# see--/speech_recognition

Hardware: AMD Instinct MI355X
Metric: 1s 16kHz clips/sec training throughput (higher is better)
Workload: dtype f32

## Files before the change

speech_recognition_amd/csrc/dw_bwd_body.h:

```cpp
#pragma once
#include "internal.h"

namespace kws_dw {

#ifndef KWS_DW_NT
#define KWS_DW_NT 1
#endif
typedef float dw_v4f __attribute__((ext_vector_type(4)));
__device__ __forceinline__ float4 ld4_stream(const float* p) {
  if (KWS_DW_NT & 2) {
    const dw_v4f v = __builtin_nontemporal_load(reinterpret_cast<const dw_v4f*>(p));
    return make_float4(v.x, v.y, v.z, v.w);
  }
  return *reinterpret_cast<const float4*>(p);
}
__device__ __forceinline__ void st4_stream(float* p, float4 o) {
  if (KWS_DW_NT & 1) {
    dw_v4f v = {o.x, o.y, o.z, o.w};
    __builtin_nontemporal_store(v, reinterpret_cast<dw_v4f*>(p));
    return;
  }
  *reinterpret_cast<float4*>(p) = o;
}

#ifndef KWS_DW_TT
#define KWS_DW_TT 8
#endif
constexpr int TT = KWS_DW_TT;

__device__ __forceinline__ float4 f4_fma(float4 a, float4 b, float4 c) {
  return make_float4(fmaf(a.x, b.x, c.x), fmaf(a.y, b.y, c.y), fmaf(a.z, b.z, c.z), fmaf(a.w, b.w, c.w));
}
__device__ __forceinline__ float4 f4_mul(float4 a, float4 b) {
  return make_float4(a.x * b.x, a.y * b.y, a.z * b.z, a.w * b.w);
}
__device__ __forceinline__ float4 f4_zero() { return make_float4(0.f, 0.f, 0.f, 0.f); }

#ifndef DW_BWD_THREADS
#define DW_BWD_THREADS 512
#endif
#ifndef DW_BWD_HT
#define DW_BWD_HT 8
#endif
#ifndef DW_BWD2_THREADS
#define DW_BWD2_THREADS 512
#endif
#ifndef DW_BWD_PARTS
#define DW_BWD_PARTS 256
#endif

struct BwdArgs {
  const float* dz; const float* y; const float* bn; const float* w; const float* coef;
  float* g; float* part;
  int B, Lin, Lout, C, pad_l, nchunks, R, Cb;
  unsigned* amax;
  int add_stride = 0, add_len = 0;
};
constexpr int bwd_smem_floats(int mode, int threads) { return mode == 2 ? 4 : 5 * threads * 4; }

template <int S, bool HAS_BN, int MODE, bool GUARD, bool ADDS = false>
__device__ __forceinline__ void bwd_body(const BwdArgs& p, float* const red, const int bid, const int nblk, const int by) {
  const float* __restrict__ dz = p.dz;
  const float* __restrict__ y = p.y;
  const float* __restrict__ bn = p.bn;
  const float* __restrict__ w = p.w;
  const float* __restrict__ coef = p.coef;
  float* __restrict__ g = p.g;
  float* __restrict__ part = p.part;
  const int B = p.B, Lin = p.Lin, Lout = p.Lout, C = p.C, pad_l = p.pad_l, nchunks = p.nchunks, R = p.R, Cb = p.Cb;
  constexpr int RSTRIDE = (MODE == 2 ? 4 : DW_BWD_THREADS * 4);
  float gmax = 0.f;
  const int C4 = Cb >> 2;
  const int tid = threadIdx.x;
  const bool live = !GUARD || tid < R * C4;
  const int r = live ? tid / C4 : 0, c4 = live ? tid - r * C4 : 0;
  const int c = by * Cb + c4 * 4;
  float4 sg = f4_zero(), sgx = f4_zero(), sw0 = f4_zero(), sw1 = f4_zero(), sw2 = f4_zero();
  float4 sc = f4_zero(), sh = f4_zero(), mean = f4_zero(), rstd = f4_zero();
  if (HAS_BN) {
    sc = *reinterpret_cast<const float4*>(bn + c);
    sh = *reinterpret_cast<const float4*>(bn + C + c);
    mean = *reinterpret_cast<const float4*>(bn + 2 * C + c);
    rstd = *reinterpret_cast<const float4*>(bn + 3 * C + c);
  }
  const float4 w0 = *reinterpret_cast<const float4*>(w + c);
  const float4 w1 = *reinterpret_cast<const float4*>(w + C + c);
  const float4 w2 = *reinterpret_cast<const float4*>(w + 2 * C + c);
  float4 c1 = f4_zero(), c2 = f4_zero();
  if (MODE == 2) {
    c1 = *reinterpret_cast<const float4*>(coef + c);
    c2 = *reinterpret_cast<const float4*>(coef + C + c);
  }
  for (int64_t ub = bid; ub * R < (int64_t)B * nchunks; ub += nblk) {
    const int64_t unit = ub * R + r;
    const int64_t b = unit / nchunks;
    const int chunk = (int)(unit - b * nchunks);
    if (b >= B || !live) continue;
    const float* yb = y + b * (int64_t)Lin * C + c;
    float* gb = g + b * (int64_t)Lin * C + c;
    const float* dzb = dz + b * (int64_t)Lout * C + c;
    const int u0 = chunk * TT;
    constexpr int HT = DW_BWD_HT;
    constexpr int ND = S == 1 ? HT + 2 : HT / 2 + 2;
    const bool podd = (pad_l & 1) != 0;
#pragma unroll
    for (int h = 0; h < TT / HT; ++h) {
      const int ub = u0 + h * HT;
      if (ub >= Lin) break;
      float4 yv[HT], D[ND];
#pragma unroll
      for (int i = 0; i < HT; ++i) yv[i] = ld4_stream(yb + (int64_t)(ub + i < Lin ? ub + i : ub) * C);
      const int t_lo = S == 1 ? ub + pad_l - 2 : ((ub + pad_l) >> 1) - 1;
#pragma unroll
      for (int j = 0; j < ND; ++j) {
        const int t = t_lo + j;
        D[j] = ld4_stream(dzb + (int64_t)(t < 0 ? 0 : (t < Lout ? t : Lout - 1)) * C);
      }
#pragma unroll
      for (int j = 0; j < ND; ++j) {
        const int t = t_lo + j;
        if (t < 0 || t >= Lout) D[j] = f4_zero();
      }
#pragma unroll
      for (int i = 0; i < HT; ++i) {
        const int u = ub + i;
        if (u >= Lin) continue;
        float4 d0, d1, d2;
        if (S == 1) {
          d0 = D[i + 2]; d1 = D[i + 1]; d2 = D[i];
        } else if ((i & 1) == 0) {
          d0 = podd ? f4_zero() : D[i / 2 + 1];
          d2 = podd ? f4_zero() : D[i / 2];
          d1 = podd ? D[i / 2 + 1] : f4_zero();
        } else {
          d0 = podd ? D[(i + 1) / 2 + 1] : f4_zero();
          d2 = podd ? D[(i + 1) / 2] : f4_zero();
          d1 = podd ? f4_zero() : D[(i - 1) / 2 + 1];
        }
        const float4 yy = yv[i];
        float4 a = yy, mk = make_float4(1.f, 1.f, 1.f, 1.f), xh = f4_zero();
        if (HAS_BN) {
          const float4 pre = make_float4(fmaf(yy.x, sc.x, sh.x), fmaf(yy.y, sc.y, sh.y), fmaf(yy.z, sc.z, sh.z),
                                         fmaf(yy.w, sc.w, sh.w));
          a = make_float4(relu6f(pre.x), relu6f(pre.y), relu6f(pre.z), relu6f(pre.w));
          mk = make_float4((pre.x > 0.f && pre.x <= 6.f) ? 1.f : 0.f, (pre.y > 0.f && pre.y <= 6.f) ? 1.f : 0.f,
                           (pre.z > 0.f && pre.z <= 6.f) ? 1.f : 0.f, (pre.w > 0.f && pre.w <= 6.f) ? 1.f : 0.f);
          xh = make_float4((yy.x - mean.x) * rstd.x, (yy.y - mean.y) * rstd.y, (yy.z - mean.z) * rstd.z,
                           (yy.w - mean.w) * rstd.w);
        }
        float4 da = f4_mul(w0, d0);
        da = f4_fma(w1, d1, da);
        da = f4_fma(w2, d2, da);
        const float4 gv = f4_mul(da, mk);
        if (MODE == 2) {
          float4 o;
          o.x = sc.x * (gv.x - c1.x - (yy.x - mean.x) * rstd.x * c2.x);
          o.y = sc.y * (gv.y - c1.y - (yy.y - mean.y) * rstd.y * c2.y);
          o.z = sc.z * (gv.z - c1.z - (yy.z - mean.z) * rstd.z * c2.z);
          o.w = sc.w * (gv.w - c1.w - (yy.w - mean.w) * rstd.w * c2.w);
          st4_stream(gb + (int64_t)u * C, o);
          gmax = kws_abs4max(gmax, o);
          continue;
        }
        if (MODE == 0) {
          float4 o = gv;
          if (coef != nullptr) {
            if (!ADDS) {
              const float4 ad = *reinterpret_cast<const float4*>(coef + (b * (int64_t)Lin + u) * C + c);
              o = make_float4(o.x + ad.x, o.y + ad.y, o.z + ad.z, o.w + ad.w);
            } else {
              const int q = u / p.add_stride;
              const bool on = q * p.add_stride == u && q < p.add_len;
              const float4 ad = *reinterpret_cast<const float4*>(coef + (b * (int64_t)p.add_len + (on ? q : 0)) * C + c);
              o = make_float4(on ? o.x + ad.x : o.x, on ? o.y + ad.y : o.y, on ? o.z + ad.z : o.z, on ? o.w + ad.w : o.w);
            }
          }
          st4_stream(gb + (int64_t)u * C, o);
        }
        sg.x += gv.x; sg.y += gv.y; sg.z += gv.z; sg.w += gv.w;
        sgx = f4_fma(gv, xh, sgx);
        sw0 = f4_fma(d0, a, sw0);
        sw1 = f4_fma(d1, a, sw1);
        sw2 = f4_fma(d2, a, sw2);
      }
    }
  }
  if (MODE == 2) {
    if (p.amax && live) kws_absmax_commit(p.amax, gmax);
    return;
  }
  if constexpr (MODE != 2) {
  if (live) {
    *reinterpret_cast<float4*>(&red[0 * RSTRIDE + tid * 4]) = sg;
    *reinterpret_cast<float4*>(&red[1 * RSTRIDE + tid * 4]) = sgx;
    *reinterpret_cast<float4*>(&red[2 * RSTRIDE + tid * 4]) = sw0;
    *reinterpret_cast<float4*>(&red[3 * RSTRIDE + tid * 4]) = sw1;
    *reinterpret_cast<float4*>(&red[4 * RSTRIDE + tid * 4]) = sw2;
  }
  __syncthreads();
  for (int o = tid; o < 5 * Cb; o += blockDim.x) {
    const int q = o / Cb, ch = o - q * Cb;
    float s = 0.f;
    for (int rr = 0; rr < R; ++rr) s += red[q * RSTRIDE + (rr * C4) * 4 + ch];
    part[((int64_t)bid * 5 + q) * C + by * Cb + ch] = s;
  }
  }
}

constexpr int KWS_DW_BWD_MAX_PARTS = DW_BWD_PARTS;
struct BwdGeom {
  int nchunks, R, block, ny, Cb;
  int64_t grid;
};
inline bool bwd_geom_ok(int C) { return C > 0 && C % 4 == 0 && (C / 4) % ceil_div(C / 4, 256) == 0; }
inline BwdGeom bwd_geom(int B, int Lin, int C, bool parts = true) {
  BwdGeom g;
  const int threads = parts ? DW_BWD_THREADS : DW_BWD2_THREADS;
  const int max_parts = parts ? KWS_DW_BWD_MAX_PARTS : 1024;
  g.ny = ceil_div(C / 4, 256);
  g.Cb = C / g.ny;
  const int C4 = g.Cb / 4;
  g.nchunks = ceil_div(Lin, TT);
  g.R = threads / C4;
  if (g.R < 1) g.R = 1;
  g.block = g.R * C4;
  g.grid = ceil_div64((int64_t)B * g.nchunks, g.R);
  if (g.grid > max_parts) g.grid = max_parts;
  return g;
}

}
```

Measured before the change: 232,200.

## Software-pipeline depthwise conv backward loads across batches

Restructures the depthwise-conv backward body so the global loads for the next tile of y and dz are issued before the current tile is consumed, using a ring of register buffers. By default this is on only for the mode-1 variant (the gradient-stats path); modes 0 and 2 keep the old loop behind macros. The goal is to hide memory latency in a streaming, bandwidth-bound kernel. In exchange it raises register pressure and can lower occupancy, and it may issue extra loads past the end of the work for tail iterations.

```diff
diff --git a/speech_recognition_amd/csrc/dw_bwd_body.h b/speech_recognition_amd/csrc/dw_bwd_body.h
--- a/speech_recognition_amd/csrc/dw_bwd_body.h
+++ b/speech_recognition_amd/csrc/dw_bwd_body.h
@@ -47,6 +47,15 @@
 #endif
 #ifndef DW_BWD_PARTS
 #define DW_BWD_PARTS 256
+#endif
+#ifndef KWS_DW_BWD_PIPE
+#define KWS_DW_BWD_PIPE 1
+#endif
+#ifndef KWS_DW_BWD0_PIPE
+#define KWS_DW_BWD0_PIPE 0
+#endif
+#ifndef KWS_DW_BWD2_PIPE
+#define KWS_DW_BWD2_PIPE 0
 #endif
 
 struct BwdArgs {
@@ -91,97 +100,167 @@
     c1 = *reinterpret_cast<const float4*>(coef + c);
     c2 = *reinterpret_cast<const float4*>(coef + C + c);
   }
-  for (int64_t ub = bid; ub * R < (int64_t)B * nchunks; ub += nblk) {
-    const int64_t unit = ub * R + r;
-    const int64_t b = unit / nchunks;
-    const int chunk = (int)(unit - b * nchunks);
-    if (b >= B || !live) continue;
+  constexpr int HT = DW_BWD_HT;
+  constexpr int NH = TT / HT;
+  constexpr int ND = S == 1 ? HT + 2 : HT / 2 + 2;
+  constexpr int PIPE = MODE == 2 ? KWS_DW_BWD2_PIPE : (MODE == 0 ? KWS_DW_BWD0_PIPE : KWS_DW_BWD_PIPE);
+  const bool podd = (pad_l & 1) != 0;
+  const int64_t units = (int64_t)B * nchunks;
+  struct Batch {
+    float4 yv[HT], D[ND];
+    int64_t b;
+    int ub;
+    bool ok;
+  };
+  auto issue = [&](Batch& q) __attribute__((always_inline)) {
+    const int64_t b = q.b;
+    const int ub = q.ub;
     const float* yb = y + b * (int64_t)Lin * C + c;
+    const float* dzb = dz + b * (int64_t)Lout * C + c;
+#pragma unroll
+    for (int i = 0; i < HT; ++i) q.yv[i] = ld4_stream(yb + (int64_t)(ub + i < Lin ? ub + i : ub) * C);
+    const int t_lo = S == 1 ? ub + pad_l - 2 : ((ub + pad_l) >> 1) - 1;
+#pragma unroll
+    for (int j = 0; j < ND; ++j) {
+      const int t = t_lo + j;
+      q.D[j] = ld4_stream(dzb + (int64_t)(t < 0 ? 0 : (t < Lout ? t : Lout - 1)) * C);
+    }
+  };
+  float4 ad[MODE == 0 && PIPE != 0 ? HT : 1];
+  auto load_add = [&](const Batch& q) __attribute__((always_inline)) {
+    if (coef == nullptr) return;
+    const int64_t b = q.b;
+    const int ub = q.ub;
+#pragma unroll
+    for (int i = 0; i < HT; ++i) {
+      const int u = ub + i < Lin ? ub + i : ub;
+      if (!ADDS) {
+        ad[i] = *reinterpret_cast<const float4*>(coef + (b * (int64_t)Lin + u) * C + c);
+      } else {
+        const int qq = u / p.add_stride;
+        const bool on = qq * p.add_stride == u && qq < p.add_len;
+        ad[i] = *reinterpret_cast<const float4*>(coef + (b * (int64_t)p.add_len + (on ? qq : 0)) * C + c);
+      }
+    }
+  };
+  auto consume = [&](Batch& q) __attribute__((always_inline)) {
+    const int64_t b = q.b;
+    const int ub = q.ub;
     float* gb = g + b * (int64_t)Lin * C + c;
-    const float* dzb = dz + b * (int64_t)Lout * C + c;
-    const int u0 = chunk * TT;
-    constexpr int HT = DW_BWD_HT;
-    constexpr int ND = S == 1 ? HT + 2 : HT / 2 + 2;
-    const bool podd = (pad_l & 1) != 0;
-#pragma unroll
-    for (int h = 0; h < TT / HT; ++h) {
-      const int ub = u0 + h * HT;
-      if (ub >= Lin) break;
-      float4 yv[HT], D[ND];
-#pragma unroll
-      for (int i = 0; i < HT; ++i) yv[i] = ld4_stream(yb + (int64_t)(ub + i < Lin ? ub + i : ub) * C);
-      const int t_lo = S == 1 ? ub + pad_l - 2 : ((ub + pad_l) >> 1) - 1;
-#pragma unroll
-      for (int j = 0; j < ND; ++j) {
-        const int t = t_lo + j;
-        D[j] = ld4_stream(dzb + (int64_t)(t < 0 ? 0 : (t < Lout ? t : Lout - 1)) * C);
-      }
-#pragma unroll
-      for (int j = 0; j < ND; ++j) {
-        const int t = t_lo + j;
-        if (t < 0 || t >= Lout) D[j] = f4_zero();
-      }
-#pragma unroll
-      for (int i = 0; i < HT; ++i) {
-        const int u = ub + i;
-        if (u >= Lin) continue;
-        float4 d0, d1, d2;
-        if (S == 1) {
-          d0 = D[i + 2]; d1 = D[i + 1]; d2 = D[i];
-        } else if ((i & 1) == 0) {
-          d0 = podd ? f4_zero() : D[i / 2 + 1];
-          d2 = podd ? f4_zero() : D[i / 2];
-          d1 = podd ? D[i / 2 + 1] : f4_zero();
-        } else {
-          d0 = podd ? D[(i + 1) / 2 + 1] : f4_zero();
-          d2 = podd ? D[(i + 1) / 2] : f4_zero();
-          d1 = podd ? f4_zero() : D[(i - 1) / 2 + 1];
+    const int t_lo = S == 1 ? ub + pad_l - 2 : ((ub + pad_l) >> 1) - 1;
+    float4 (&yv)[HT] = q.yv;
+    float4 (&D)[ND] = q.D;
+#pragma unroll
+    for (int j = 0; j < ND; ++j) {
+      const int t = t_lo + j;
+      if (t < 0 || t >= Lout) D[j] = f4_zero();
+    }
+#pragma unroll
+    for (int i = 0; i < HT; ++i) {
+      const int u = ub + i;
+      if (u >= Lin) continue;
+      float4 d0, d1, d2;
+      if (S == 1) {
+        d0 = D[i + 2]; d1 = D[i + 1]; d2 = D[i];
+      } else if ((i & 1) == 0) {
+        d0 = podd ? f4_zero() : D[i / 2 + 1];
+        d2 = podd ? f4_zero() : D[i / 2];
+        d1 = podd ? D[i / 2 + 1] : f4_zero();
+      } else {
+        d0 = podd ? D[(i + 1) / 2 + 1] : f4_zero();
+        d2 = podd ? D[(i + 1) / 2] : f4_zero();
+        d1 = podd ? f4_zero() : D[(i - 1) / 2 + 1];
+      }
+      const float4 yy = yv[i];
+      float4 a = yy, mk = make_float4(1.f, 1.f, 1.f, 1.f), xh = f4_zero();
+      if (HAS_BN) {
+        const float4 pre = make_float4(fmaf(yy.x, sc.x, sh.x), fmaf(yy.y, sc.y, sh.y), fmaf(yy.z, sc.z, sh.z),
+                                       fmaf(yy.w, sc.w, sh.w));
+        a = make_float4(relu6f(pre.x), relu6f(pre.y), relu6f(pre.z), relu6f(pre.w));
+        mk = make_float4((pre.x > 0.f && pre.x <= 6.f) ? 1.f : 0.f, (pre.y > 0.f && pre.y <= 6.f) ? 1.f : 0.f,
+                         (pre.z > 0.f && pre.z <= 6.f) ? 1.f : 0.f, (pre.w > 0.f && pre.w <= 6.f) ? 1.f : 0.f);
+        xh = make_float4((yy.x - mean.x) * rstd.x, (yy.y - mean.y) * rstd.y, (yy.z - mean.z) * rstd.z,
+                         (yy.w - mean.w) * rstd.w);
+      }
+      float4 da = f4_mul(w0, d0);
+      da = f4_fma(w1, d1, da);
+      da = f4_fma(w2, d2, da);
+      const float4 gv = f4_mul(da, mk);
+      if (MODE == 2) {
+        float4 o;
+        o.x = sc.x * (gv.x - c1.x - (yy.x - mean.x) * rstd.x * c2.x);
+        o.y = sc.y * (gv.y - c1.y - (yy.y - mean.y) * rstd.y * c2.y);
+        o.z = sc.z * (gv.z - c1.z - (yy.z - mean.z) * rstd.z * c2.z);
+        o.w = sc.w * (gv.w - c1.w - (yy.w - mean.w) * rstd.w * c2.w);
+        st4_stream(gb + (int64_t)u * C, o);
+        gmax = kws_abs4max(gmax, o);
+        continue;
+      }
+      if (MODE == 0) {
+        float4 o = gv;
+        if (coef != nullptr) {
+          if (!ADDS) {
+            const float4 av = PIPE != 0 ? ad[i] : *reinterpret_cast<const float4*>(coef + (b * (int64_t)Lin + u) * C + c);
+            o = make_float4(o.x + av.x, o.y + av.y, o.z + av.z, o.w + av.w);
+          } else {
+            const int qq = u / p.add_stride;
+            const bool on = qq * p.add_stride == u && qq < p.add_len;
+            const float4 av = PIPE != 0 ? ad[i]
+                                        : *reinterpret_cast<const float4*>(coef + (b * (int64_t)p.add_len + (on ? qq : 0)) * C + c);
+            o = make_float4(on ? o.x + av.x : o.x, on ? o.y + av.y : o.y, on ? o.z + av.z : o.z, on ? o.w + av.w : o.w);
+          }
         }
-        const float4 yy = yv[i];
-        float4 a = yy, mk = make_float4(1.f, 1.f, 1.f, 1.f), xh = f4_zero();
-        if (HAS_BN) {
-          const float4 pre = make_float4(fmaf(yy.x, sc.x, sh.x), fmaf(yy.y, sc.y, sh.y), fmaf(yy.z, sc.z, sh.z),
-                                         fmaf(yy.w, sc.w, sh.w));
-          a = make_float4(relu6f(pre.x), relu6f(pre.y), relu6f(pre.z), relu6f(pre.w));
-          mk = make_float4((pre.x > 0.f && pre.x <= 6.f) ? 1.f : 0.f, (pre.y > 0.f && pre.y <= 6.f) ? 1.f : 0.f,
-                           (pre.z > 0.f && pre.z <= 6.f) ? 1.f : 0.f, (pre.w > 0.f && pre.w <= 6.f) ? 1.f : 0.f);
-          xh = make_float4((yy.x - mean.x) * rstd.x, (yy.y - mean.y) * rstd.y, (yy.z - mean.z) * rstd.z,
-                           (yy.w - mean.w) * rstd.w);
-        }
-        float4 da = f4_mul(w0, d0);
-        da = f4_fma(w1, d1, da);
-        da = f4_fma(w2, d2, da);
-        const float4 gv = f4_mul(da, mk);
-        if (MODE == 2) {
-          float4 o;
-          o.x = sc.x * (gv.x - c1.x - (yy.x - mean.x) * rstd.x * c2.x);
-          o.y = sc.y * (gv.y - c1.y - (yy.y - mean.y) * rstd.y * c2.y);
-          o.z = sc.z * (gv.z - c1.z - (yy.z - mean.z) * rstd.z * c2.z);
-          o.w = sc.w * (gv.w - c1.w - (yy.w - mean.w) * rstd.w * c2.w);
-          st4_stream(gb + (int64_t)u * C, o);
-          gmax = kws_abs4max(gmax, o);
-          continue;
-        }
-        if (MODE == 0) {
-          float4 o = gv;
-          if (coef != nullptr) {
-            if (!ADDS) {
-              const float4 ad = *reinterpret_cast<const float4*>(coef + (b * (int64_t)Lin + u) * C + c);
-              o = make_float4(o.x + ad.x, o.y + ad.y, o.z + ad.z, o.w + ad.w);
-            } else {
-              const int q = u / p.add_stride;
-              const bool on = q * p.add_stride == u && q < p.add_len;
-              const float4 ad = *reinterpret_cast<const float4*>(coef + (b * (int64_t)p.add_len + (on ? q : 0)) * C + c);
-              o = make_float4(on ? o.x + ad.x : o.x, on ? o.y + ad.y : o.y, on ? o.z + ad.z : o.z, on ? o.w + ad.w : o.w);
-            }
-          }
-          st4_stream(gb + (int64_t)u * C, o);
-        }
-        sg.x += gv.x; sg.y += gv.y; sg.z += gv.z; sg.w += gv.w;
-        sgx = f4_fma(gv, xh, sgx);
-        sw0 = f4_fma(d0, a, sw0);
-        sw1 = f4_fma(d1, a, sw1);
-        sw2 = f4_fma(d2, a, sw2);
+        st4_stream(gb + (int64_t)u * C, o);
+      }
+      sg.x += gv.x; sg.y += gv.y; sg.z += gv.z; sg.w += gv.w;
+      sgx = f4_fma(gv, xh, sgx);
+      sw0 = f4_fma(d0, a, sw0);
+      sw1 = f4_fma(d1, a, sw1);
+      sw2 = f4_fma(d2, a, sw2);
+    }
+  };
+  if constexpr (PIPE == 0) {
+    for (int64_t ub = bid; ub * R < units; ub += nblk) {
+      const int64_t unit = ub * R + r;
+      const int64_t b = unit / nchunks;
+      const int chunk = (int)(unit - b * nchunks);
+      if (b >= B || !live) continue;
+      const int u0 = chunk * TT;
+#pragma unroll
+      for (int h = 0; h < NH; ++h) {
+        Batch q;
+        q.b = b;
+        q.ub = u0 + h * HT;
+        if (q.ub >= Lin) break;
+        issue(q);
+        consume(q);
+      }
+    }
+  } else {
+    constexpr int NB = PIPE + 1;
+    Batch q[NB];
+    int64_t ubn = bid;
+    int hn = 0;
+    auto issue_next = [&](Batch& nx) __attribute__((always_inline)) {
+      const int64_t unit = ubn * R + r;
+      const int64_t b = unit / nchunks;
+      const int ub = (int)(unit - b * nchunks) * TT + hn * HT;
+      nx.ok = live && b < B && ub < Lin;
+      nx.b = nx.ok ? b : 0;
+      nx.ub = nx.ok ? ub : 0;
+      issue(nx);
+      if (++hn == NH) { hn = 0; ubn += nblk; }
+    };
+    const int64_t nub = (units + R - 1) / R;
+    const int64_t n = bid < nub ? ((nub - 1 - bid) / nblk + 1) * NH : 0;
+#pragma unroll
+    for (int j = 0; j < PIPE; ++j) issue_next(q[j]);
+    for (int64_t k = 0; k < n; k += NB) {
+#pragma unroll
+      for (int j = 0; j < NB; ++j) {
+        if (MODE == 0) load_add(q[j]);
+        issue_next(q[(j + PIPE) % NB]);
+        if (q[j].ok) consume(q[j]);
       }
     }
   }
```

New measurement: 230,800. Within noise of the previous version (-0.6%).
